# termuxinator/html5-canvas-raytracer

Measured on AMD Instinct MI355X. Metric: Mpixel/s, higher is better.
Workload: dtype f64; 1 GPU; cfg3: h8 scene (8 spheres, 2 lights, depth 3, supersample 1) at 3840x2160; SCENE, CAMERA AND LAUNCH TABLE RESIDENT (a static frame rendered again and again: cold_frame / new_camera_every_step are the other cases); one launch per frame; kernel=fma

## Files before the change

### html5-canvas-raytracer_amd/csrc/rt_api.hip

```cpp

#include "rt_api_internal.h"
#include "rt_wide.h"

namespace rt_api {

thread_local char g_err[512] = "";

int fail(int code, const char *fmt, ...) {
  va_list ap;
  va_start(ap, fmt);
  vsnprintf(g_err, sizeof g_err, fmt, ap);
  va_end(ap);
  return code;
}

lib_state G;

int ensure_device(int d) {
  if (!G.inited) return fail(RT_ERR_STATE, "rt_init has not been called");
  if (d < 0 || d >= (int)G.dev.size()) return fail(RT_ERR_INVALID, "device %d out of range (0..%d)", d, (int)G.dev.size() - 1);
  device_state &s = G.dev[d];
  HIP_TRY(hipSetDevice(s.hip_id));
  std::lock_guard<std::mutex> lk(G.dev_mu);
  if (!s.stream) {
    hipStream_t st = nullptr;
    HIP_TRY(hipMalloc(&s.d_counters, 7 * sizeof(unsigned long long)));
    HIP_TRY(hipMemset(s.d_counters, 0, 7 * sizeof(unsigned long long)));
    HIP_TRY(hipStreamCreateWithFlags(&st, hipStreamNonBlocking));
    s.stream = st;
  }
  return RT_OK;
}

int device_stream(int device, void *hip_stream, hipStream_t *stream) {
  if (int rc = ensure_device(device)) return rc;
  *stream = hip_stream ? (hipStream_t)hip_stream : G.dev[device].stream;
  return RT_OK;
}

int scratch_guard(device_state &D, hipStream_t stream, size_t per_lane, uint64_t waves_in_grid, const char *what) {
#ifdef RT_TESTING
  bool pretend = false;
  if (const char *q = getenv("RT_TEST_SCRATCH_PER_LANE")) { per_lane = (size_t)strtoull(q, nullptr, 10); pretend = true; }
#else
  const bool pretend = false;
#endif
  if (per_lane == 0) return RT_OK;
  std::lock_guard<std::mutex> lk(G.dev_mu);
  if (!pretend) for (const device_state::scratch_seen &c : D.scratch_checked) if (c.stream == stream && c.per_lane >= per_lane) return RT_OK;
  if (!D.wave_slots) {
    hipDeviceProp_t p;
    HIP_TRY(hipGetDeviceProperties(&p, D.hip_id));
    D.wave_slots = (size_t)p.multiProcessorCount * (size_t)(p.maxThreadsPerMultiProcessor / 64);
    if (!D.wave_slots) D.wave_slots = 8192;
  }
  const uint64_t slots = waves_in_grid < D.wave_slots ? waves_in_grid : D.wave_slots;
  const uint64_t reservation = (uint64_t)per_lane * 64u * slots;
  size_t free_b = 0, total_b = 0;
  HIP_TRY(hipMemGetInfo(&free_b, &total_b));
  const uint64_t margin = (uint64_t)64 << 20;
// ... 371 lines not shown
```

### html5-canvas-raytracer_amd/csrc/rt_kernel.hip

```cpp

#include <hip/hip_runtime.h>
#include <math.h>
#include <stdint.h>

#include "rt_device.h"
#include "rt_block.h"
#include "rt_wide.h"

#ifndef RT_STRICT
#define RT_STRICT 0
#endif
#if RT_STRICT
#define RT_LAUNCH_NAME rt_launch_trace_strict
#define RT_SCRATCH_NAME rt_scratch_trace_strict
#else
#define RT_LAUNCH_NAME rt_launch_trace_fast
#define RT_SCRATCH_NAME rt_scratch_trace_fast
#endif

#ifndef RT_WAVES_PER_EU
#define RT_WAVES_PER_EU 2
#endif

constexpr unsigned rt_waves_per_eu(bool refract, bool grid, bool w1) {
// ... 125 lines not shown
#if RT_STRICT
  const v3 target = mk(o.x + L.cam_axis_x[0] * d0 + L.cam_axis_y[0] * d0 + L.cam_axis_z[0] * d0,
                       o.y + L.cam_axis_x[1] * d1 + L.cam_axis_y[1] * d1 + L.cam_axis_z[1] * d1,
                       o.z + L.cam_axis_x[2] * d2 + L.cam_axis_y[2] * d2 + L.cam_axis_z[2] * d2);
  const v3 ray = unit(mk(target.x - o.x, target.y - o.y, target.z - o.z), &rl);
#else
  const v3 rawray = mk(L.cam_axis_sum[0] * d0, L.cam_axis_sum[1] * d1, L.ray_bias[2]);
  rl = rt_rsqrt_pos(dot(rawray, rawray));
  const v3 ray = mk(rawray.x * rl, rawray.y * rl, rawray.z * rl);
#endif

#ifdef RT_TESTING
  const bool is_probe = L.probe != nullptr && sx == L.probe_x && sy == L.probe_y && blockIdx.z == 0;
#else
  const bool is_probe = false;
#endif
  const auto stage_finish = [&](const uint32_t tid) __attribute__((always_inline)) {
    if constexpr (!IMAGE_IN_LDS) {
    } else if constexpr (GRID || W1) {
      rt_u4 *lds4 = (rt_u4 *)lds_raw;
      const rt_u4 *__restrict__ image4 = (const rt_u4 *)L.lds_image;
#pragma unroll
      for (uint32_t i = 0; i < RT_STAGE_PIECES; i++) {
        const uint32_t k = tid + i * KT;
        if (i * KT < image_vec && k < image_vec) lds4[k] = piece[i];
      }
      for (uint32_t k = tid + RT_STAGE_PIECES * KT; k < image_vec; k += KT) lds4[k] = image4[k];
    } else {
      if (tid < image_words) lds_raw[tid] = stage0;
      for (uint32_t k = tid + RT_WG_THREADS; k < image_words; k += RT_WG_THREADS) lds_raw[k] = image[k];
    }
  };
  [[maybe_unused]] bool uni_done = false;
  if constexpr (UNI_OK) {
    if (RT_UNI_TRY()) {
      uni_done = trace_pixel<REFRACT, COUNT, GRID, SS2, false, W1, true>(L, (const rt_mtl *)L.lds_image, (const rt_texture_desc *)((const double *)L.lds_image + mtl_words), acc,
                                                                         cull_lds, cull0, lane, 0.0, 0.0, 0.0, 0.0, o, ray, rgb, cnt, is_probe, P0.cand | (cell << 24));
      if (!uni_done) {
        uint32_t tid4 = threadIdx.x;
        if constexpr (MTL_ONLY) tid4 = rt_lane_again(); else
        asm volatile("" : "+v"(tid4));
        stage_issue(tid4);
        stage_finish(tid4);
      }
#ifdef RT_TESTING
      else if (lane == 0u && L.uniform_waves != nullptr) {
        atomicAdd(L.uniform_waves, 1ull);
        if (cell & 1u) atomicAdd(L.uniform_waves + 1, 1ull);
      }
#endif
    }
  }
  if (!uni_done) {
    if (!UNI_OK || !RT_UNI_TRY()) stage_finish(tid);
    if constexpr (IMAGE_IN_LDS) __syncthreads();

    const double bw = SS2 ? 15.0 : 7.0, bh = SS2 ? 3.0 : 7.0;
    const double lx = SS2 ? (double)(2u * ((lane >> 2) & 7u) + (sub & 1u)) : (double)(lane & 7u);
    const double ly = SS2 ? (double)(2u * (lane >> 5) + (sub >> 1)) : (double)(lane >> 3);
    double blk_x0 = 0.0, blk_x1 = 0.0, blk_y0 = 0.0, blk_y1 = 0.0;
    if (!UNI_OK || !RT_UNI_TRY()) { blk_x0 = d0 - lx; blk_x1 = blk_x0 + bw; blk_y1 = d1 + ly; blk_y0 = blk_y1 - bh; }
    trace_pixel<REFRACT, COUNT, GRID, SS2, false, W1>(L, mtl, tex, acc, cull_lds, cull0, lane, blk_x0, blk_x1, blk_y0, blk_y1, o, ray, rgb, cnt, is_probe, P0.cand);
  }
  }
#undef RT_UNI_TRY

  uint32_t tid2 = threadIdx.x;
  if constexpr (W1 && !GRID) tid2 = rt_lane_again(); else
  asm volatile("" : "+v"(tid2));
  const rt_pixel P1 = rt_pixel_of<SS2, W1>(L, tid2);
#if !RT_STRICT
  const uint32_t wide = rt_cold_args()->wide_stores;
  asm volatile("" :: "s"(wide), "s"(L.scatter), "s"(L.rgb24), "s"(L.w), "s"(L.out), "s"(L.frame_stride));
#endif
  const uint32_t frame_i = blockIdx.z;
  const bool valid = P1.valid;
  if constexpr (WAVE_FLAGS) { if (P1.sky) { rgb[0] = L.sky_rgb[0]; rgb[1] = L.sky_rgb[1]; rgb[2] = L.sky_rgb[2]; } }
  const uint32_t r8 = to_byte(rgb[0]), g8 = to_byte(rgb[1]), b8 = to_byte(rgb[2]);
#if RT_STRICT
  uint32_t *__restrict__ out = L.scatter ? L.out_frames[frame_i] : L.out + (size_t)frame_i * L.frame_stride;
  const uint32_t orow = L.scatter ? P1.frow : P1.lrow;
#endif
  uint32_t rgbw;
  if (!SS2) rgbw = r8 | (g8 << 8) | (b8 << 16);
  else {
    uint32_t packed = r8 | (g8 << 10) | (b8 << 20);
    packed += __shfl_xor(packed, 1);
    packed += __shfl_xor(packed, 2);
    rgbw = (((packed & 1023u) + 2u) >> 2) | ((((packed >> 10) & 1023u) + 2u) >> 2 << 8) | ((((packed >> 20) & 1023u) + 2u) >> 2 << 16);
  }
#if RT_STRICT
  const uint32_t n_run = 1u;
#else
  const uint32_t n_run = P1.sky ? P1.run : 1u;
#endif
// ... 255 lines not shown
```

### html5-canvas-raytracer_amd/csrc/rt_kernel_trace.h

```cpp

#include "rt_uniform_pred.h"

#define RT_PIN() asm volatile("")
#define RT_ROOT(TCA, DISC)                                                                    \
        const double thc_ = rt_sqrt_nn<REFRACT>(DISC);                                                 \
        const double t0_ = (TCA) - thc_, t1_ = (TCA) + thc_;                                  \
        const bool in_ = (t0_ < eps);                                                         \
        const double t_ = in_ ? t1_ : t0_;
#define RT_CAND(IDX, TCA, DISC)                                                               \
      if (!((DISC) < 0.0)) {                                                                  \
        RT_PIN();                                                                             \
        RT_ROOT(TCA, DISC)                                                                    \
        const bool closer_ = (t_ < ht) && !(t_ < eps);              \
        ht = closer_ ? t_ : ht;                                                               \
        hcode = closer_ ? ((int)(2u * (IDX)) + (in_ ? 1 : 0)) : hcode;                        \
      }
#define RT_GENERIC(IDX, G)                                                                    \
      {                                                                                       \
        const v3 Lv_ = mk((G).ox - p.x, (G).oy - p.y, (G).oz - p.z);                          \
        const double tca_ = dot(d, Lv_);                                                      \
        const double disc_ = (G).r2 - (dot(Lv_, Lv_) - tca_ * tca_);                          \
        RT_CAND(IDX, tca_, disc_)                                                             \
      }
#define RT_ANCHORED_DISC(G)                                                                   \
// ... 91 lines not shown
              }                                                                               \
            }
__device__ __forceinline__ bool rt_nonzero_scalar(double x) {
  unsigned long long b_ = __builtin_bit_cast(unsigned long long, x);
  asm volatile("" : "+s"(b_));
  return rt_nonzero_bits(b_);
}
#define RT_OA4_NONZERO(X) (SIX_FORMS ? rt_nonzero_scalar(X) : ((X) != 0.0))
#define RT_SHADOW_U(J, G)                                                                     \
            {                                                                               \
              RT_SDISC(G, tc_, disc_)                                                       \
              if (((int)(J) != hi) && !(disc_ < 0.0)) {                                     \
                RT_PIN();                                                                   \
                const double thc_ = rt_sqrt_nn<REFRACT>(disc_);                                      \
                RT_SROOTS(tc_, thc_, t0_, t1_)                                              \
                const double t_ = (t0_ < eps) ? t1_ : t0_;                                  \
                if ((t_ < llen) && !(t_ < eps) && li != 0.0) {                              \
                  RT_PIN();                                                                 \
                  const double oa4_ = objs[J].albedo[4];                                    \
                  li = RT_OA4_NONZERO(oa4_) ? rt_div(li, oa4_) : 0.0;                       \
                }                                                                           \
              }                                                                             \
            }

#define RT_CHAIN_END()                                                                                                          \
        if constexpr (SIX_WAVES) {                                                                                              \
          if (map_valid) {                                                                                                      \
            const double S_ = acc[0];                                                                                           \
            _Pragma("unroll")                                                                                                   \
            for (int c = 0; c < 3; c++) ret[c] = rt_max_nn(acc[(4 + c) * 64u], rt_min_nn(acc[(7 + c) * 64u], __builtin_fma(S_, ret[c], acc[(1 + c) * 64u])));   \
          }                                                                                                                     \
        }

template <bool REFRACT, bool COUNT, bool GRID, bool SS2, bool ITEM = false, bool W1 = false, bool UNI = false>
__device__ __forceinline__ bool trace_pixel(const rt_launch &L, const rt_mtl *mtl, const rt_texture_desc *tex,
                                            [[maybe_unused]] double *acc, [[maybe_unused]] const rt_geom *cull_lds, [[maybe_unused]] const rt_geom cull0, [[maybe_unused]] uint32_t lane,
                                            [[maybe_unused]] double blk_x0, [[maybe_unused]] double blk_x1, [[maybe_unused]] double blk_y0,
                                            [[maybe_unused]] double blk_y1, v3 p, v3 d, double rgb[3], uint32_t cnt[3],
                                            [[maybe_unused]] bool is_probe, [[maybe_unused]] uint32_t cand_host,
                                            [[maybe_unused]] uint32_t own_sx = 0u, [[maybe_unused]] uint32_t own_sy = 0u, [[maybe_unused]] uint32_t own_f = 0u) {
  static_assert(!UNI || (W1 && !REFRACT && !COUNT && !ITEM && !RT_STRICT), "uniform-material path: the one-wave-workgroup product kernels");
#ifdef RT_TESTING
  uint32_t probe_n = 0;
  double probe_li = 0.0;
#endif
  const sphere_kptr objs = (sphere_kptr)L.objects;
  const geom_kptr geom = (geom_kptr)L.geom;
  const uint32_t N = L.n_objects, NL = L.n_lights;
  const double eps = L.epsilon;
  const uint32_t NLOOP = L.n_loop;
  const uint32_t enc = L.enclosing;
  const bool cull_lds_on = (!RT_STRICT && !COUNT) ? (!GRID && !W1) : (L.cull_in_lds != 0u);
#if RT_STRICT
  constexpr bool FOLD_FORWARD = false;
#else
  constexpr bool FOLD_FORWARD = true;
#endif
  constexpr bool LEAN = !RT_STRICT && !REFRACT && !COUNT && !ITEM;
  [[maybe_unused]] constexpr bool SIX_FORMS = LEAN && W1 && !GRID;
  [[maybe_unused]] frame<REFRACT> stack[FOLD_FORWARD ? 1 : RT_MAX_SEGS];
  [[maybe_unused]] park parked[(FOLD_FORWARD && REFRACT) ? RT_MAX_SEGS : 1];
  [[maybe_unused]] int sp = 0;
  [[maybe_unused]] bool map_valid = false;
  int level = 0;
  [[maybe_unused]] uint32_t tree_path = 1u;
#if defined(RT_TESTING) && defined(RT_ABLATE_BOUNCE)
  uint32_t segs_left = L.segs ? 1 : 0;
#else
  uint32_t segs_left = L.segs;
#endif
  double ret[3] = {0.0, 0.0, 0.0};
  constexpr bool SIX_WAVES = FOLD_FORWARD && W1 && !GRID && !REFRACT && !COUNT && !ITEM && !UNI;
  constexpr bool WAVE_NODE = LEAN && !GRID && !UNI;
  [[maybe_unused]] uint32_t turn = 0u;

  double ht = RT_INF; int hcode = -1;
  if constexpr (UNI) { if (segs_left == 0) return false; }
  if (segs_left != 0) {
        [[maybe_unused]] const geom_kptr ga = (geom_kptr)L.geom_cam;
#if !RT_STRICT
        if constexpr (UNI) {
          const uint32_t i = cand_host & 255u;
          const rt_geom g0 = rt_load_geom32(ga, i);
          typename rt_mtl_src<true>::type &mu = *rt_mtl_at<true>(mtl, i);
          if ((mu.albedo[3] > 0.0 && segs_left > 1) || rt_mtl_kind(mu) == RT_SAMPLER_STARS) return false;
          RT_ANCHORED_DISC(g0)
          const double t0_ = tca_ - rt_sqrt_nn<REFRACT>(disc_);
          const bool met_ = !(disc_ < 0.0) && (t0_ < ht) && !(t0_ < eps);
          if (__ballot(!met_) != 0ull) return false;
#if defined(RT_TESTING) && defined(RT_ABLATE_UNIFORM)
          rgb[0] = rgb[1] = rgb[2] = 0.0;
          return true;
#endif
          ht = t0_; hcode = (int)(2u * i);
        } else
        if (cand_host != 0u) {
          { const uint32_t i = cand_host & 255u; const rt_geom g0 = rt_load_geom32(ga, i); RT_ANCHORED(i, g0) }
          if (cand_host >= (2u << 16)) { const uint32_t i = (cand_host >> 8) & 255u; const rt_geom g0 = rt_load_geom32(ga, i); RT_ANCHORED(i, g0) }
        } else
#endif
        for (uint32_t base = 0; base < NLOOP; base += 64u) {
          const uint32_t j = base + lane;
          const uint32_t jj = j < NLOOP ? j : 0u;
          double c0 = cull0.ox, c1 = cull0.oy, c2 = cull0.oz, c3 = cull0.r2;
          if constexpr (ITEM) {
          } else if (cull_lds_on) {
            const rt_geom __attribute__((address_space(3))) *g = (const rt_geom __attribute__((address_space(3))) *)cull_lds + jj;
            c0 = g->ox; c1 = g->oy; c2 = g->oz; c3 = g->r2;
          } else if (base != 0u || (W1 && !GRID)) {
            const rt_geom __attribute__((address_space(1))) *g = (const rt_geom __attribute__((address_space(1))) *)L.cull + jj;
            c0 = g->ox; c1 = g->oy; c2 = g->oz; c3 = g->r2;
          }
          const rt_geom cr = rt_geom{c0, c1, c2, c3};
          unsigned long long m = __ballot(j < NLOOP) & __ballot(cr.ox * L.proj_d <= blk_x1) & __ballot(cr.oy * L.proj_d >= blk_x0) &
                                 __ballot(cr.oz * L.proj_d <= blk_y1) & __ballot(cr.r2 * L.proj_d >= blk_y0);
          if constexpr (ITEM) m = (NLOOP - base >= 64u) ? ~0ull : ((1ull << (NLOOP - base)) - 1ull);
          while (m) {
            const uint32_t i = base + (uint32_t)__builtin_ctzll(m);
            m &= m - 1ull;
#if RT_STRICT
            const rt_geom g0 = rt_load_geom32(geom, i);
            RT_GENERIC(i, g0)
#else
            const rt_geom g0 = rt_load_geom32(ga, i);
            RT_ANCHORED(i, g0)
#endif
          }
        }
  }
  bool searched = true;
  [[maybe_unused]] bool first_bounce = false;
#if !RT_STRICT
  if (!UNI && L.sky_fast && segs_left != 0 && __ballot(hcode >= 0) == 0ull) {
    if (COUNT) { cnt[0]++; cnt[2] += N; }
    rgb[0] = L.sky_rgb[0]; rgb[1] = L.sky_rgb[1]; rgb[2] = L.sky_rgb[2];
    return true;
  }
#endif

  if (segs_left != 0) {
    for (;;) {
      [[maybe_unused]] const uint32_t node_no = turn;
      if constexpr (WAVE_NODE) {
        turn++;
        searched = (node_no == 0u); first_bounce = (node_no == 1u); map_valid = (node_no != 0u);
      }
      if (COUNT) cnt[0]++;
      if (!UNI && !searched) {
        bool scanned = false;
#if !RT_STRICT
        if constexpr (GRID) {
          if (rt_cold_args()->bounce_table != nullptr) {
            const uint32_t from = (uint32_t)(hcode >> 1);
            const double ax = __builtin_fabs(d.x), ay = __builtin_fabs(d.y), az = __builtin_fabs(d.z);
            const bool bx = (ax >= ay) && (ax >= az), by = !bx && (ay >= az);
            const double dm = bx ? d.x : (by ? d.y : d.z);
            const double du = bx ? d.y : d.x, dv = (bx || by) ? d.z : d.y;
            const double sc = (0.5 * RT_BGRID) * __builtin_amdgcn_rcp(__builtin_fabs(dm));
            const double fu = __builtin_fmin(__builtin_fmax(__builtin_fma(du, sc, 0.5 * RT_BGRID), 0.0), (double)(RT_BGRID - 1u));
            const double fv = __builtin_fmin(__builtin_fmax(__builtin_fma(dv, sc, 0.5 * RT_BGRID), 0.0), (double)(RT_BGRID - 1u));
            const uint32_t face = (bx ? 0u : (by ? 2u : 4u)) + ((dm < 0.0) ? 1u : 0u);
            const uint32_t key = from * RT_BCELLS + face * (RT_BGRID * RT_BGRID) + (uint32_t)fv * RT_BGRID + (uint32_t)fu;
            const uint32_t words = (NLOOP + 63u) >> 6;
            ht = RT_INF; hcode = -1;
            for (uint32_t wd = 0; wd < words; wd++) {
              unsigned long long cand = 0ull, todo = __ballot(true);
// ... 84 lines not shown
        { const auto &mc = RT_COLD(miss_color); ret[0] = mc[0]; ret[1] = mc[1]; ret[2] = mc[2]; }
#ifdef RT_TESTING
        if (is_probe && probe_n < RT_PROBE_NODES) {
          double *q = L.probe + (size_t)(probe_n++) * RT_PROBE_WORDS;
          for (uint32_t z = 0; z < RT_PROBE_WORDS; z++) q[z] = 0.0;
          q[0] = (double)(REFRACT ? tree_path : (1u << rt_lvl(level))); q[1] = -1.0; q[2] = ht; q[9] = d.x; q[10] = d.y; q[11] = d.z;
          q[17] = (double)segs_left; q[19] = p.x; q[20] = p.y; q[21] = p.z; q[23] = 1.0;
        }
#endif
        RT_CHAIN_END()
      } else {
        typename rt_mtl_src<UNI>::type &m = *rt_mtl_at<UNI>(mtl, (uint32_t)hi);
        const v3 h = mk(p.x + d.x * ht, p.y + d.y * ht, p.z + d.z * ht);
#if RT_STRICT
        double nlen;
        const v3 n = unit(mk(h.x - m.origin[0], h.y - m.origin[1], h.z - m.origin[2]), &nlen);
#else
        const double inv_r = m.inv_r;
        const v3 n = mk((h.x - m.origin[0]) * inv_r, (h.y - m.origin[1]) * inv_r, (h.z - m.origin[2]) * inv_r);
#endif
        v3 l;
        if constexpr (UNI) l = n;
        else l = inside ? mk(-n.x, -n.y, -n.z) : n;
        double a0 = m.albedo[0];
        const double a1 = m.albedo[1], a2 = m.albedo[2];
        double a3 = m.albedo[3];
        const double a4 = REFRACT ? m.albedo[4] : 0.0;
#if !RT_STRICT && !defined(RT_ABLATE_QAMP)
        if (!UNI && ((WAVE_NODE ? node_no != 0u : rt_lvl(level) != 0) || ((a3 > 0.0 || a4 > 0.0) && segs_left > 1))) {
          const float ir_ = (float)inv_r;
          const float q_ = RT_Q_OF(RT_Q_GET(level), (float)ht, ir_, __builtin_fabsf((float)dot(d, n)), rt_r_get(level));
          level = rt_q_put(level, q_);
          level = rt_r_put(level, __builtin_amdgcn_rcpf(ir_));
        }
#endif

        double col[3];
#if defined(RT_TESTING) && defined(RT_ABLATE_SAMPLER)
        const int kind = RT_SAMPLER_COLOR;
#else
        const int kind = rt_mtl_kind(m);
#endif
#if RT_STRICT
        if (kind == RT_SAMPLER_TEXTURE) {
          double t_at, t_as;
          rt_atan2_asin<REFRACT>(-n.z, -n.x, -n.y, &t_at, &t_as);
          const double u = RT_DIV_CONST(t_at, M_PI) / 2.0 + 0.5;
          const double v = RT_DIV_CONST(t_as, M_PI / 2.0) / 2.0 + 0.5;
          const rt_texture_desc td = rt_tex_desc<UNI>(tex, rt_mtl_texture(m));
          const double xd = ceil(u * (double)td.width) - 1.0, yd = ceil(v * (double)td.height) - 1.0;
          uint32_t xi = (xd > 0.0) ? (uint32_t)xd : 0u, yi = (yd > 0.0) ? (uint32_t)yd : 0u;
          xi = min(xi, td.width - 1u); yi = min(yi, td.height - 1u);
          const uint32_t texel = *(const uint32_t *)(L.texel_base + td.texels_offset + ((size_t)yi * td.width + xi) * 4u);
          col[0] = RT_DIV_CONST((double)(texel & 255u), 255.0); col[1] = RT_DIV_CONST((double)((texel >> 8) & 255u), 255.0);
          col[2] = RT_DIV_CONST((double)((texel >> 16) & 255u), 255.0);
          if (xd != xd || yd != yd) col[0] = col[1] = col[2] = __builtin_nan("");
        } else if (kind == RT_SAMPLER_CHECKER) {
          double t_at, t_as;
          rt_atan2_asin<REFRACT>(-n.y, -n.x, -n.z, &t_at, &t_as);
          const double u = RT_DIV_CONST(t_at, M_PI) / 2.0 + 0.5;
          const double v = RT_DIV_CONST(t_as, M_PI / 2.0) / 2.0 + 0.5;
          const int c = to_int32_bit0(u * m.c[6]) ^ to_int32_bit0(v * m.c[7]);
          col[0] = m.c[3 * c]; col[1] = m.c[3 * c + 1]; col[2] = m.c[3 * c + 2];
#else
        [[maybe_unused]] double t_at, t_as;
        [[maybe_unused]] const bool one_cell = UNI && !GRID && kind == RT_SAMPLER_CHECKER && (cand_host & (1u << 24)) != 0u;
// ... 247 lines not shown
        }

#if RT_STRICT
        const v3 nq = n;
#else
        const v3 nq = inside ? mk(-l.x, -l.y, -l.z) : l;
#endif
        v3 r = mk(0, 0, 0); double rlen = 0.0;
#if !RT_STRICT
        if constexpr (LEAN) { if (!UNI && a3 > 0.0 && segs_left > 1) r = unit_go(reflect(d, l), &rlen); } else
#endif
        if (!UNI && a3 > 0.0 && segs_left > 1) r = unit(reflect(d, nq), &rlen);
        v3 f = mk(0, 0, 0); double flen = 0.0;
        if (REFRACT && a4 > 0.0 && segs_left > 1) {
          const double dn = dot(d, nq);
          double cosi = -((dn < -1.0) ? -1.0 : min1(dn));
          v3 nn = nq; double eta;
          if (cosi < 0.0) { cosi = -cosi; nn = mk(-nq.x, -nq.y, -nq.z); eta = m.refract_index; }
          else eta = rt_rcp(m.refract_index);
          const double k = 1.0 - eta * eta * (1.0 - cosi * cosi);
          if (k > 0.0) {
            const double q = eta * cosi - rt_sqrt(k);
            f = mk(d.x * eta + nn.x * q, d.y * eta + nn.y * q, d.z * eta + nn.z * q);
          } else f = reflect(d, nn);
          f = unit(f, &flen);
        }

        if constexpr (FOLD_FORWARD && REFRACT) {
#pragma unroll
          for (int c = 0; c < 3; c++) col[c] = acc[(10 + c) * RT_WG_THREADS];
        }
        const bool go_r = !UNI && (rlen != 0.0);
        const bool go_f = REFRACT && (flen != 0.0);
#ifdef RT_TESTING
        if (is_probe && probe_n < RT_PROBE_NODES) {
          double *q = L.probe + (size_t)(probe_n++) * RT_PROBE_WORDS;
          q[0] = (double)(REFRACT ? tree_path : (1u << rt_lvl(level))); q[1] = (double)hcode; q[2] = ht;
          q[3] = h.x; q[4] = h.y; q[5] = h.z; q[6] = n.x; q[7] = n.y; q[8] = n.z; q[9] = d.x; q[10] = d.y; q[11] = d.z;
          q[12] = col[0]; q[13] = col[1]; q[14] = col[2]; q[15] = diffuse; q[16] = specular; q[17] = (double)segs_left;
          q[18] = probe_li; q[19] = p.x; q[20] = p.y; q[21] = p.z; q[22] = (double)(go_r ? 1 : 0) + 2.0 * (go_f ? 1 : 0); q[23] = 1.0;
        }
#endif
        if (!go_r && !go_f) {
          if constexpr (UNI) {
            double x[3];
#pragma unroll
            for (int c = 0; c < 3; c++) x[c] = col[c] * diffuse + col[c] * specular;
            const double poison = (((draw + sraw) + x[0]) + x[1]) + x[2];
            if (__ballot(poison != poison) == 0ull) {
#pragma unroll
              for (int c = 0; c < 3; c++) ret[c] = rt_max_nn(col[c] * a0, rt_min1_nn(x[c]));
            } else {
#if defined(RT_TESTING) && defined(RT_ABLATE_LIGHT)
              const bool lit = false;
#else
              const bool lit = (a1 > 0.0 || a2 > 0.0);
#endif
              const double d2 = lit ? min1(draw) * a1 : 0.0, s2 = lit ? min1(sraw) * a2 : 0.0;
#pragma unroll
              for (int c = 0; c < 3; c++) ret[c] = maxa(col[c] * a0, min1(col[c] * d2 + col[c] * s2));
            }
          } else {
#pragma unroll
          for (int c = 0; c < 3; c++) ret[c] = maxa(col[c] * a0, min1(col[c] * diffuse + col[c] * specular));
          RT_CHAIN_END()
          }
// ... 30 lines not shown
                if constexpr (LEAN) {
                  const double l2 = __builtin_fma(S, A[c], O), h2 = __builtin_fma(S, rt_max1_nn(A[c]), O);
                  acc[(1 + c) * T] = __builtin_fma(S, D[c], O);
                  acc[(4 + c) * T] = rt_max_nn(LO, rt_min_nn(HI, l2));
                  acc[(7 + c) * T] = rt_max_nn(LO, rt_min_nn(HI, h2));
                } else {
                const double l2 = __builtin_fma(S, A[c], O), h2 = __builtin_fma(S, __builtin_fmax(A[c], 1.0), O);
                acc[(1 + c) * T] = __builtin_fma(S, D[c], O);
                acc[(4 + c) * T] = __builtin_fmax(LO, __builtin_fmin(HI, l2));
                acc[(7 + c) * T] = __builtin_fmax(LO, __builtin_fmin(HI, h2));
                }
              }
              acc[0] = S * coef;
            }
            if constexpr (!WAVE_NODE) map_valid = true;
            p = h; d = via_f ? f : r; tree_path = 2u * tree_path + (via_f ? 1u : 0u);
          }
          level++; segs_left--;
          descend = true;
        } else {
          frame<REFRACT> &fr = stack[level];
#pragma unroll
          for (int c = 0; c < 3; c++) { fr.amb[c] = col[c] * a0; fr.ds[c] = col[c] * diffuse + col[c] * specular; }
          fr.a3 = a3;
          if constexpr (REFRACT) {
            fr.a4 = a4; fr.h[0] = h.x; fr.h[1] = h.y; fr.h[2] = h.z; fr.f[0] = f.x; fr.f[1] = f.y; fr.f[2] = f.z;
            fr.re[0] = fr.re[1] = fr.re[2] = 0.0;
            fr.has_f = go_f; fr.phase = go_r ? 0 : 1;
          }
          p = h; d = go_r ? r : f;
          tree_path = 2u * tree_path + (go_r ? 0u : 1u);
          level++; segs_left--;
          descend = true;
        }
      }
      if (descend) continue;

      if constexpr (SIX_WAVES) break;
      else if constexpr (FOLD_FORWARD) {
        const uint32_t T = W1 ? 64u : RT_WG_THREADS;
        if (map_valid) {
          const double S = acc[0];
#pragma unroll
          for (int c = 0; c < 3; c++) {
            if constexpr (LEAN) ret[c] = rt_max_nn(acc[(4 + c) * T], rt_min_nn(acc[(7 + c) * T], __builtin_fma(S, ret[c], acc[(1 + c) * T])));
            else ret[c] = __builtin_fmax(acc[(4 + c) * T], __builtin_fmin(acc[(7 + c) * T], __builtin_fma(S, ret[c], acc[(1 + c) * T])));
          }
        }
        bool resumed = false;
        if constexpr (REFRACT) {
          if (sp > 0) {
            const park &pk = parked[--sp];
            const double coef = pk.a4;
            if (!pk.map_valid) {
              acc[0] = coef;
#pragma unroll
              for (int c = 0; c < 3; c++) {
                acc[(1 + c) * T] = pk.ds[c] + ret[c] * pk.a3; acc[(4 + c) * T] = pk.amb[c]; acc[(7 + c) * T] = __builtin_fmax(pk.amb[c], 1.0);
              }
            } else {
              const double S = pk.S;
#pragma unroll
              for (int c = 0; c < 3; c++) {
                const double Dn = pk.ds[c] + ret[c] * pk.a3;
                const double l2 = __builtin_fma(S, pk.amb[c], pk.O[c]), h2 = __builtin_fma(S, __builtin_fmax(pk.amb[c], 1.0), pk.O[c]);
                acc[(1 + c) * T] = __builtin_fma(S, Dn, pk.O[c]);
// ... 63 lines not shown
```

### html5-canvas-raytracer_amd/csrc/rt_launch.hip

```cpp

#include "rt_api_internal.h"

extern "C" int rt_render_tiles_device(rt_scene_dev *s, uint32_t w, uint32_t h, const rt_tiles *tiles, void *d_out, void *hip_stream,
                                      uint32_t flags, rt_stats *stats) {
  return rt_render_batch_device(s, w, h, tiles, 1u, d_out, 0u, hip_stream, flags, stats);
}

namespace {
int render_batch_impl(rt_scene_dev *s, uint32_t w, uint32_t h, const rt_tiles *tiles, uint32_t n_frames, void *d_out, uint64_t frame_stride_bytes,
                      void *const *d_frames, void *hip_stream, uint32_t flags, rt_stats *stats, uint32_t ss_override = 0u);
#ifdef RT_TESTING
thread_local struct { double *d_buf; uint32_t x, y; } g_probe = {nullptr, 0u, 0u};
#endif

void bind_scene_order(const rt_scene_dev *s, rt_launch &K) {
  const uint8_t *ob = obj_block(s);
  K.objects = (const rt_sphere *)(ob + s->o_objs);
  K.geom = (const rt_geom *)(ob + s->o_geom);
  K.lds_image = lds_image_of(s);
  K.n_loop = s->hd.n_objects;
  K.enclosing = ~0u;
  memcpy(K.miss_color, s->hd.miss_color, sizeof K.miss_color);
}
}
// ... 33 lines not shown
  return RT_OK;
}
extern "C" int rt_test_cell_waves(int device, unsigned long long *out_waves) {
  if (!out_waves) return fail(RT_ERR_INVALID, "rt_test_cell_waves: NULL argument");
  int rc = ensure_device(device);
  if (rc) return rc;
  device_state &D = G.dev[device];
  HIP_TRY(hipSetDevice(D.hip_id));
  HIP_TRY(hipDeviceSynchronize());
  HIP_TRY(hipMemcpy(out_waves, D.d_counters + 4, sizeof *out_waves, hipMemcpyDeviceToHost));
  HIP_TRY(hipMemset(D.d_counters + 4, 0, sizeof *out_waves));
  return RT_OK;
}
extern "C" int rt_test_first_bounce_waves(int device, unsigned long long *out_waves) {
  if (!out_waves) return fail(RT_ERR_INVALID, "rt_test_first_bounce_waves: NULL argument");
  int rc = ensure_device(device);
  if (rc) return rc;
  device_state &D = G.dev[device];
  HIP_TRY(hipSetDevice(D.hip_id));
  HIP_TRY(hipDeviceSynchronize());
  HIP_TRY(hipMemcpy(out_waves, D.d_counters + 5, sizeof *out_waves, hipMemcpyDeviceToHost));
  HIP_TRY(hipMemset(D.d_counters + 5, 0, sizeof *out_waves));
  return RT_OK;
}
extern "C" int rt_test_second_node_waves(int device, unsigned long long *out_waves) {
  if (!out_waves) return fail(RT_ERR_INVALID, "rt_test_second_node_waves: NULL argument");
  int rc = ensure_device(device);
  if (rc) return rc;
  device_state &D = G.dev[device];
  HIP_TRY(hipSetDevice(D.hip_id));
  HIP_TRY(hipDeviceSynchronize());
  HIP_TRY(hipMemcpy(out_waves, D.d_counters + 6, sizeof *out_waves, hipMemcpyDeviceToHost));
  HIP_TRY(hipMemset(D.d_counters + 6, 0, sizeof *out_waves));
  return RT_OK;
}
#endif

extern "C" int rt_render_batch_device(rt_scene_dev *s, uint32_t w, uint32_t h, const rt_tiles *tiles, uint32_t n_frames, void *d_out,
                                      uint64_t frame_stride_bytes, void *hip_stream, uint32_t flags, rt_stats *stats) {
  if (!d_out) return fail(RT_ERR_INVALID, "NULL scene, tiles or output");
  return render_batch_impl(s, w, h, tiles, n_frames, d_out, frame_stride_bytes, nullptr, hip_stream, flags, stats);
}

extern "C" int rt_render_scatter_device(rt_scene_dev *s, uint32_t w, uint32_t h, const rt_tiles *tiles, uint32_t n_frames, void *const *d_frames,
                                        void *hip_stream, uint32_t flags, rt_stats *stats) {
  if (!d_frames) return fail(RT_ERR_INVALID, "NULL frame pointer array");
  if (n_frames == 0 || n_frames > RT_MAX_SCATTER) return fail(RT_ERR_INVALID, "scatter: n_frames %u not in 1..%u", n_frames, RT_MAX_SCATTER);
  if (flags & RT_FLAG_RGB24) return fail(RT_ERR_INVALID, "scatter writes whole RGBA8 frames: RT_FLAG_RGB24 does not apply");
  for (uint32_t f = 0; f < n_frames; f++) if (!d_frames[f] || ((uintptr_t)d_frames[f] & 3u)) return fail(RT_ERR_INVALID, "scatter: frame pointer %u is NULL or unaligned", f);
  return render_batch_impl(s, w, h, tiles, n_frames, nullptr, 0u, d_frames, hip_stream, flags, stats);
}

namespace {
struct rt_box_launch {
  const uint32_t *src; uint64_t src_frame_stride;
  uint32_t *out; uint64_t frame_stride; uint32_t *out_frames[RT_MAX_SCATTER]; uint32_t scatter;
  uint32_t w, h, band_rows, tile_rows, tile_first, tile_stride;
};
template <uint32_t K>
__global__ void __launch_bounds__(256) rt_box_filter_kernel(const rt_box_launch B) {
  const uint32_t x = blockIdx.x * 256u + threadIdx.x, f = blockIdx.z;
  if (x >= B.w) return;
  const uint32_t *__restrict__ src = B.src + (size_t)f * B.src_frame_stride;
  for (uint32_t lrow = blockIdx.y; lrow < B.band_rows; lrow += gridDim.y) {
    const uint32_t tile_i = lrow / B.tile_rows, trow = lrow - tile_i * B.tile_rows;
    const uint32_t frow = (B.tile_first + tile_i * B.tile_stride) * B.tile_rows + trow;
// ... 804 lines not shown
```

Measured before the change: 179,800 Mpixel/s.

## Let uniform-material waves hit mirrors and hand off reflection to general path

Before this change, the uniform-material fast path gave up whenever a wave hit a reflective sphere, and the whole first hit was redone on the general path. Now the fast path shades the first hit and stores the hit point, the reflected ray, the level and the accumulator state in a handover struct. The general trace then resumes at the bounce and skips the primary intersection search. LDS staging is issued from inside the fast path so it overlaps the shading. This adds code and registers, plus the risk that occupancy drops or the shaded result differs from the general path.

```diff
diff --git a/html5-canvas-raytracer_amd/csrc/rt_api.hip b/html5-canvas-raytracer_amd/csrc/rt_api.hip
--- a/html5-canvas-raytracer_amd/csrc/rt_api.hip
+++ b/html5-canvas-raytracer_amd/csrc/rt_api.hip
@@ -24,8 +24,8 @@
   std::lock_guard<std::mutex> lk(G.dev_mu);
   if (!s.stream) {
     hipStream_t st = nullptr;
-    HIP_TRY(hipMalloc(&s.d_counters, 7 * sizeof(unsigned long long)));
-    HIP_TRY(hipMemset(s.d_counters, 0, 7 * sizeof(unsigned long long)));
+    HIP_TRY(hipMalloc(&s.d_counters, 8 * sizeof(unsigned long long)));
+    HIP_TRY(hipMemset(s.d_counters, 0, 8 * sizeof(unsigned long long)));
     HIP_TRY(hipStreamCreateWithFlags(&st, hipStreamNonBlocking));
     s.stream = st;
   }
diff --git a/html5-canvas-raytracer_amd/csrc/rt_kernel.hip b/html5-canvas-raytracer_amd/csrc/rt_kernel.hip
--- a/html5-canvas-raytracer_amd/csrc/rt_kernel.hip
+++ b/html5-canvas-raytracer_amd/csrc/rt_kernel.hip
@@ -181,14 +181,36 @@
     }
   };
   [[maybe_unused]] bool uni_done = false;
+  [[maybe_unused]] rt_handover ho;
+  ho.state = 0u;
+  [[maybe_unused]] uint32_t uw = 0u;
+  [[maybe_unused]] const auto uw_bit = [&](const uint32_t b) __attribute__((always_inline)) { uint32_t w_ = uw; asm volatile("" : "+s"(w_)); return (w_ & b) != 0u; };
   if constexpr (UNI_OK) {
     if (RT_UNI_TRY()) {
+      if constexpr (WAVE_FLAGS) {
+#pragma unroll
+        for (uint32_t i = 0; i < RT_STAGE_PIECES; i++) asm volatile("" : "=v"(piece[i]));
+        const auto stage_now = [&]() __attribute__((always_inline)) { stage_issue(rt_lane_again()); };
+        uni_done = trace_pixel<REFRACT, COUNT, GRID, SS2, false, W1, true, decltype(stage_now)>(L, (const rt_mtl *)L.lds_image, (const rt_texture_desc *)((const double *)L.lds_image + mtl_words), acc,
+                                                                           cull_lds, cull0, lane, 0.0, 0.0, 0.0, 0.0, o, ray, rgb, cnt, is_probe, P0.cand | (cell << 24), 0u, 0u, 0u, &ho, stage_now);
+      } else
       uni_done = trace_pixel<REFRACT, COUNT, GRID, SS2, false, W1, true>(L, (const rt_mtl *)L.lds_image, (const rt_texture_desc *)((const double *)L.lds_image + mtl_words), acc,
                                                                          cull_lds, cull0, lane, 0.0, 0.0, 0.0, 0.0, o, ray, rgb, cnt, is_probe, P0.cand | (cell << 24));
-      if (!uni_done) {
+      if constexpr (WAVE_FLAGS) {
+        uw = (uint32_t)__builtin_amdgcn_readfirstlane((int)((ho.state & 1u) != 0u ? ho.state : (uni_done ? 4u : 0u)));
+        asm volatile("" : "+s"(uw));
+        ho.state = uw;
+      }
+      if (WAVE_FLAGS ? !uw_bit(4u) : !uni_done) {
         uint32_t tid4 = threadIdx.x;
         if constexpr (MTL_ONLY) tid4 = rt_lane_again(); else
         asm volatile("" : "+v"(tid4));
+        if constexpr (WAVE_FLAGS) {
+          if (!uw_bit(1u)) { RT_PIN(); stage_issue(tid4); }
+#ifdef RT_TESTING
+          if (uw_bit(2u) && lane == 0u && L.uniform_waves != nullptr) atomicAdd(L.uniform_waves + 4, 1ull);
+#endif
+        } else
         stage_issue(tid4);
         stage_finish(tid4);
       }
@@ -200,16 +222,28 @@
 #endif
     }
   }
-  if (!uni_done) {
+  if (WAVE_FLAGS ? !uw_bit(4u) : !uni_done) {
+    double blk_x0 = 0.0, blk_x1 = 0.0, blk_y0 = 0.0, blk_y1 = 0.0;
+    if constexpr (WAVE_FLAGS) {
+      if (!RT_UNI_TRY()) {
+        stage_finish(tid);
+        const double bw = SS2 ? 15.0 : 7.0, bh = SS2 ? 3.0 : 7.0;
+        const double lx = SS2 ? (double)(2u * ((lane >> 2) & 7u) + (sub & 1u)) : (double)(lane & 7u);
+        const double ly = SS2 ? (double)(2u * (lane >> 5) + (sub >> 1)) : (double)(lane >> 3);
+        blk_x0 = d0 - lx; blk_x1 = blk_x0 + bw; blk_y1 = d1 + ly; blk_y0 = blk_y1 - bh;
+      }
+      if constexpr (IMAGE_IN_LDS) __syncthreads();
+    } else {
     if (!UNI_OK || !RT_UNI_TRY()) stage_finish(tid);
     if constexpr (IMAGE_IN_LDS) __syncthreads();
 
     const double bw = SS2 ? 15.0 : 7.0, bh = SS2 ? 3.0 : 7.0;
     const double lx = SS2 ? (double)(2u * ((lane >> 2) & 7u) + (sub & 1u)) : (double)(lane & 7u);
     const double ly = SS2 ? (double)(2u * (lane >> 5) + (sub >> 1)) : (double)(lane >> 3);
-    double blk_x0 = 0.0, blk_x1 = 0.0, blk_y0 = 0.0, blk_y1 = 0.0;
     if (!UNI_OK || !RT_UNI_TRY()) { blk_x0 = d0 - lx; blk_x1 = blk_x0 + bw; blk_y1 = d1 + ly; blk_y0 = blk_y1 - bh; }
-    trace_pixel<REFRACT, COUNT, GRID, SS2, false, W1>(L, mtl, tex, acc, cull_lds, cull0, lane, blk_x0, blk_x1, blk_y0, blk_y1, o, ray, rgb, cnt, is_probe, P0.cand);
+    }
+    trace_pixel<REFRACT, COUNT, GRID, SS2, false, W1>(L, mtl, tex, acc, cull_lds, cull0, lane, blk_x0, blk_x1, blk_y0, blk_y1, o, ray, rgb, cnt, is_probe, P0.cand,
+                                                      0u, 0u, 0u, WAVE_FLAGS ? &ho : nullptr);
   }
   }
 #undef RT_UNI_TRY
diff --git a/html5-canvas-raytracer_amd/csrc/rt_kernel_trace.h b/html5-canvas-raytracer_amd/csrc/rt_kernel_trace.h
--- a/html5-canvas-raytracer_amd/csrc/rt_kernel_trace.h
+++ b/html5-canvas-raytracer_amd/csrc/rt_kernel_trace.h
@@ -147,13 +147,17 @@
           }                                                                                                                     \
         }
 
-template <bool REFRACT, bool COUNT, bool GRID, bool SS2, bool ITEM = false, bool W1 = false, bool UNI = false>
+struct rt_handover { v3 h, r; int level; uint32_t state; uint32_t probe_n; };
+struct rt_no_stage { __device__ __forceinline__ void operator()() const {} };
+
+template <bool REFRACT, bool COUNT, bool GRID, bool SS2, bool ITEM = false, bool W1 = false, bool UNI = false, class STAGE = rt_no_stage>
 __device__ __forceinline__ bool trace_pixel(const rt_launch &L, const rt_mtl *mtl, const rt_texture_desc *tex,
                                             [[maybe_unused]] double *acc, [[maybe_unused]] const rt_geom *cull_lds, [[maybe_unused]] const rt_geom cull0, [[maybe_unused]] uint32_t lane,
                                             [[maybe_unused]] double blk_x0, [[maybe_unused]] double blk_x1, [[maybe_unused]] double blk_y0,
                                             [[maybe_unused]] double blk_y1, v3 p, v3 d, double rgb[3], uint32_t cnt[3],
                                             [[maybe_unused]] bool is_probe, [[maybe_unused]] uint32_t cand_host,
-                                            [[maybe_unused]] uint32_t own_sx = 0u, [[maybe_unused]] uint32_t own_sy = 0u, [[maybe_unused]] uint32_t own_f = 0u) {
+                                            [[maybe_unused]] uint32_t own_sx = 0u, [[maybe_unused]] uint32_t own_sy = 0u, [[maybe_unused]] uint32_t own_f = 0u,
+                                            [[maybe_unused]] rt_handover *ho = nullptr, [[maybe_unused]] STAGE stage = STAGE()) {
   static_assert(!UNI || (W1 && !REFRACT && !COUNT && !ITEM && !RT_STRICT), "uniform-material path: the one-wave-workgroup product kernels");
 #ifdef RT_TESTING
   uint32_t probe_n = 0;
@@ -173,6 +177,9 @@
 #endif
   constexpr bool LEAN = !RT_STRICT && !REFRACT && !COUNT && !ITEM;
   [[maybe_unused]] constexpr bool SIX_FORMS = LEAN && W1 && !GRID;
+  [[maybe_unused]] constexpr bool MIRROR = UNI && SIX_FORMS;
+  [[maybe_unused]] uint32_t spawn_w = 0u;
+  [[maybe_unused]] const auto spawn = [&]() __attribute__((always_inline)) { uint32_t w_ = spawn_w; asm volatile("" : "+s"(w_)); return (w_ & 1u) != 0u; };
   [[maybe_unused]] frame<REFRACT> stack[FOLD_FORWARD ? 1 : RT_MAX_SEGS];
   [[maybe_unused]] park parked[(FOLD_FORWARD && REFRACT) ? RT_MAX_SEGS : 1];
   [[maybe_unused]] int sp = 0;
@@ -191,13 +198,29 @@
 
   double ht = RT_INF; int hcode = -1;
   if constexpr (UNI) { if (segs_left == 0) return false; }
-  if (segs_left != 0) {
+  uint32_t search_segs = segs_left;
+  if constexpr (SIX_WAVES) {
+    if (ho != nullptr) {
+      if (((uint32_t)__builtin_amdgcn_readfirstlane((int)ho->state) & 2u) != 0u) {
+        turn = 1u; p = ho->h; d = ho->r; hcode = (int)(2u * (cand_host & 255u)); level = ho->level; segs_left -= 1u; search_segs = 0u;
+#ifdef RT_TESTING
+        probe_n = ho->probe_n;
+#endif
+      }
+    }
+  }
+  if (search_segs != 0) {
         [[maybe_unused]] const geom_kptr ga = (geom_kptr)L.geom_cam;
 #if !RT_STRICT
         if constexpr (UNI) {
           const uint32_t i = cand_host & 255u;
           const rt_geom g0 = rt_load_geom32(ga, i);
           typename rt_mtl_src<true>::type &mu = *rt_mtl_at<true>(mtl, i);
+          if constexpr (MIRROR) {
+            if (rt_mtl_kind(mu) == RT_SAMPLER_STARS) return false;
+            if (mu.albedo[3] > 0.0 && segs_left > 1) { RT_PIN(); spawn_w = 1u; cand_host &= ~(0x11u << 24); }
+            asm volatile("" : "+s"(spawn_w));
+          } else
           if ((mu.albedo[3] > 0.0 && segs_left > 1) || rt_mtl_kind(mu) == RT_SAMPLER_STARS) return false;
           RT_ANCHORED_DISC(g0)
           const double t0_ = tca_ - rt_sqrt_nn<REFRACT>(disc_);
@@ -246,7 +269,20 @@
   bool searched = true;
   [[maybe_unused]] bool first_bounce = false;
 #if !RT_STRICT
-  if (!UNI && L.sky_fast && segs_left != 0 && __ballot(hcode >= 0) == 0ull) {
+  if constexpr (SIX_WAVES) {
+    uint32_t sky_segs = search_segs;
+#if !(defined(RT_TESTING) && defined(RT_ABLATE_BOUNCE))
+    asm volatile("" : "+s"(sky_segs));
+#endif
+    if (L.sky_fast) {
+      RT_PIN();
+      if (sky_segs != 0) {
+        RT_PIN();
+        if (__ballot(hcode >= 0) == 0ull) { rgb[0] = L.sky_rgb[0]; rgb[1] = L.sky_rgb[1]; rgb[2] = L.sky_rgb[2]; return true; }
+      }
+    }
+  } else
+  if (!UNI && L.sky_fast && search_segs != 0 && __ballot(hcode >= 0) == 0ull) {
     if (COUNT) { cnt[0]++; cnt[2] += N; }
     rgb[0] = L.sky_rgb[0]; rgb[1] = L.sky_rgb[1]; rgb[2] = L.sky_rgb[2];
     return true;
@@ -397,6 +433,13 @@
           const float q_ = RT_Q_OF(RT_Q_GET(level), (float)ht, ir_, __builtin_fabsf((float)dot(d, n)), rt_r_get(level));
           level = rt_q_put(level, q_);
           level = rt_r_put(level, __builtin_amdgcn_rcpf(ir_));
+        }
+        if constexpr (MIRROR) {
+          if (spawn()) {
+            const float ir_ = (float)inv_r;
+            const float q_ = RT_Q_OF(RT_Q_GET(level), (float)ht, ir_, __builtin_fabsf((float)dot(d, n)), rt_r_get(level));
+            *(int *)(acc + 64u) = rt_r_put(rt_q_put(level, q_), __builtin_amdgcn_rcpf(ir_));
+          }
         }
 #endif
 
@@ -710,6 +753,41 @@
         }
         const bool go_r = !UNI && (rlen != 0.0);
         const bool go_f = REFRACT && (flen != 0.0);
+#if !RT_STRICT
+        if (MIRROR && spawn()) {
+          RT_PIN();
+          {
+            stage();
+            ho->state = 1u;
+            double rlen_;
+            const v3 r_ = unit_go(reflect(d, l), &rlen_);
+            const double poison_ = draw + sraw;
+            if (__ballot(rlen_ == 0.0 || poison_ != poison_) == 0ull) {
+#ifdef RT_TESTING
+            if (is_probe && probe_n < RT_PROBE_NODES) {
+              double *q = L.probe + (size_t)(probe_n++) * RT_PROBE_WORDS;
+              q[0] = 1.0; q[1] = (double)hcode; q[2] = ht;
+              q[3] = h.x; q[4] = h.y; q[5] = h.z; q[6] = n.x; q[7] = n.y; q[8] = n.z; q[9] = d.x; q[10] = d.y; q[11] = d.z;
+              q[12] = col[0]; q[13] = col[1]; q[14] = col[2]; q[15] = diffuse; q[16] = specular; q[17] = (double)segs_left;
+              q[18] = probe_li; q[19] = p.x; q[20] = p.y; q[21] = p.z; q[22] = 1.0; q[23] = 1.0;
+            }
+            ho->probe_n = probe_n;
+#endif
+            uint32_t slot_ = 64u;
+            asm volatile("" : "+s"(slot_));
+            const int level_ = *(const int *)(acc + slot_);
+            acc[0] = a3;
+#pragma unroll
+            for (int c = 0; c < 3; c++) {
+              const double A_ = col[c] * a0, D_ = col[c] * diffuse + col[c] * specular;
+              acc[(1 + c) * 64u] = D_; acc[(4 + c) * 64u] = A_; acc[(7 + c) * 64u] = rt_max1_nn(A_);
+            }
+            ho->h = h; ho->r = r_; ho->level = level_ + 1; ho->state = 3u;
+            }
+          }
+        } else
+#endif
+        {
 #ifdef RT_TESTING
         if (is_probe && probe_n < RT_PROBE_NODES) {
           double *q = L.probe + (size_t)(probe_n++) * RT_PROBE_WORDS;
@@ -806,6 +884,7 @@
           tree_path = 2u * tree_path + (go_r ? 0u : 1u);
           level++; segs_left--;
           descend = true;
+        }
         }
       }
       if (descend) continue;
diff --git a/html5-canvas-raytracer_amd/csrc/rt_launch.hip b/html5-canvas-raytracer_amd/csrc/rt_launch.hip
--- a/html5-canvas-raytracer_amd/csrc/rt_launch.hip
+++ b/html5-canvas-raytracer_amd/csrc/rt_launch.hip
@@ -89,6 +89,17 @@
   HIP_TRY(hipDeviceSynchronize());
   HIP_TRY(hipMemcpy(out_waves, D.d_counters + 6, sizeof *out_waves, hipMemcpyDeviceToHost));
   HIP_TRY(hipMemset(D.d_counters + 6, 0, sizeof *out_waves));
+  return RT_OK;
+}
+extern "C" int rt_test_mirror_waves(int device, unsigned long long *out_waves) {
+  if (!out_waves) return fail(RT_ERR_INVALID, "rt_test_mirror_waves: NULL argument");
+  int rc = ensure_device(device);
+  if (rc) return rc;
+  device_state &D = G.dev[device];
+  HIP_TRY(hipSetDevice(D.hip_id));
+  HIP_TRY(hipDeviceSynchronize());
+  HIP_TRY(hipMemcpy(out_waves, D.d_counters + 7, sizeof *out_waves, hipMemcpyDeviceToHost));
+  HIP_TRY(hipMemset(D.d_counters + 7, 0, sizeof *out_waves));
   return RT_OK;
 }
 #endif
diff --git a/profiles/count_mirror_blocks.py b/profiles/count_mirror_blocks.py
--- /dev/null
+++ b/profiles/count_mirror_blocks.py
@@ -0,0 +1,84 @@
+import ctypes as C
+import json
+import os
+import sys
+
+import numpy as np
+
+ROOT = os.path.dirname(os.path.dirname(os.path.abspath(__file__)))
+sys.path.insert(0, os.path.join(ROOT, "html5-canvas-raytracer_amd"))
+sys.path.insert(0, os.path.join(ROOT, "profiles"))
+import rt_host
+from count_first_bounce import table
+
+FLAGS = 1 | 2 | 4 | 32 | 128 | 256 | 512
+
+
+def count(lib, scene, w, h):
+    sys.path.insert(0, os.path.join(ROOT, "tests"))
+    import oracle_util as ou
+    c = ou.c_oracle()
+    c.oracle_probe_sample.restype = C.c_int
+    c.oracle_probe_sample.argtypes = [C.c_void_p, C.c_size_t, C.c_uint32, C.c_uint32, C.c_uint32, C.c_uint32, C.c_void_p]
+    blob = rt_host.flatten_scene(scene)
+    buf = C.create_string_buffer(blob, len(blob))
+    ss = scene.get("supersample", 1)
+    loop = [i for i, o in enumerate(scene["objects"]) if o["r2"] != 25000000]
+    tab = table(lib, blob, w, h, FLAGS)
+    live = tab[((tab[:, 0] >> 11) & 15 != 0) & (tab[:, 1] >> 31 == 0)]
+    one = live[(live[:, 3] & 0x3ffff) >> 16 == 1]
+    rec = np.zeros(64 * 24)
+    nodes = rec.reshape(64, 24)
+    out = {"live_entries": len(live), "one_candidate_entries": len(one), "spawning_waves": 0, "eligible_waves": 0, "whole_waves": 0,
+           "sky_waves": 0, "horizon_waves": 0, "inside_waves": 0, "other_hit_waves": 0, "no_descent_waves": 0}
+    for w0, w1, _, w3 in one:
+        obj = loop[int(w3) & 255]
+        if not (scene["objects"][obj]["mtl"]["albedo"][3] > 0 and scene["segs"] > 1):
+            continue
+        tile_x, rows_valid, frow0 = int(w0) & 2047, (int(w0) >> 11) & 15, int(w0) >> 15
+        sky = (int(w3) >> 31) == 1 and ((int(w1) >> 24) & 4) != 0
+        for col in range(4):
+            n = miss = inside = other = stay = 0
+            for sy in range(frow0 * ss, (frow0 + rows_valid) * ss):
+                for sx in range((tile_x * 32 + col * 8) * ss, min((tile_x * 32 + col * 8 + 8) * ss, w * ss)):
+                    rec[:] = 0.0
+                    assert c.oracle_probe_sample(buf, len(blob), w, h, sx, sy, rec.ctypes.data) == 0
+                    root = nodes[(nodes[:, 23] == 1.0) & (nodes[:, 0] == 1.0)]
+                    n += 1
+                    code = int(root[0, 1]) if len(root) else -1
+                    if code < 0 or (code >> 1) not in loop:
+                        miss += 1
+                    elif (code >> 1) != obj:
+                        other += 1
+                    elif code & 1:
+                        inside += 1
+                    elif not (int(root[0, 22]) & 1):
+                        stay += 1
+            if not n:
+                continue
+            out["spawning_waves"] += 1
+            out["horizon_waves"] += 1 if miss else 0
+            out["inside_waves"] += 1 if inside else 0
+            out["other_hit_waves"] += 1 if other else 0
+            out["no_descent_waves"] += 1 if stay else 0
+            if not (miss or inside or other or stay):
+                out["eligible_waves"] += 1
+                out["whole_waves"] += 1 if n == 64 else 0
+                out["sky_waves"] += 1 if sky else 0
+    return out
+
+
+def report(lib, name, w, h):
+    print(name, w, h, json.dumps(count(lib, rt_host.load_scene(name), w, h)), flush=True)
+
+
+if __name__ == "__main__":
+    lib = rt_host.load_library()
+    args = sys.argv[1:]
+    if args[:1] == ["--frames"]:
+        for w, h in ((3840, 2160), (7680, 4320), (1001, 563)):
+            report(lib, "h8", w, h)
+        sys.exit(0)
+    name = args[0] if args else "h8"
+    w, h = (int(args[1]), int(args[2])) if len(args) > 2 else (3840, 2160)
+    report(lib, name, w, h)
```

Result: slower. 172,500 Mpixel/s (-4.1%).
